# jpe17/TwoTowerMLRetrieval

Hardware: AMD Instinct MI355X
Metric: queries/sec top-k over 10M x 256-d docs (higher is better)
Workload: dtype f32 results (bit-identical to the fp32 FMA chain); f16-MFMA screen + fp32 rescoring; 1 GPU; exact cosine top-10 of B=1024 queries over 10000000 x 256 fp32 unit-norm passages resident in HBM (BASELINE configs[3]; configs[1] batch), row-sharded over 1 GPU(s), screened path (f16-MFMA filter + exact fp32 rescoring, bit-identical to the fp32 kernel); n_docs=10000000, dim=256, batch=1024, k=10, parallelism=rowshard1

## Files before the change

twotowermlretrieval_amd/csrc/screen.hip:

```cpp
#include "score_topk.h"
#include "keep_word.h"
#include <cmath>

#include <hip/hip_fp16.h>
#include <limits.h>
#include <math.h>

namespace {

typedef _Float16 h8 __attribute__((ext_vector_type(8)));
typedef _Float16 h4 __attribute__((ext_vector_type(4)));
typedef unsigned u32x4 __attribute__((ext_vector_type(4)));
typedef __attribute__((address_space(3))) void lds_void;
typedef const __attribute__((address_space(1))) void gbl_void;

#ifndef TT_SCREEN_STAGGER
#define TT_SCREEN_STAGGER 1
#endif
constexpr int SW = 8;
constexpr int STILE_BYTES = 32 * 512;
constexpr int SRING = 8;
constexpr int STPB = 2;
constexpr int SCAP = 128;
constexpr int SURV_MAX = 1024;
constexpr int POOL_MAX = 8192;
constexpr int FIN_MAX_CHUNKS = 2048;

struct SCand {
    float v;
    int x;
};

__device__ __forceinline__ float screen_eps(float qnorm, float dmax)
{
    return 1.10e-3f * qnorm * dmax + 1e-6f * (qnorm + dmax);
}

template <int NCH>
__device__ __forceinline__ void bf16_to_f16_lds(char *base, int lane)
{
    uint4 v[NCH];
#pragma unroll
    for (int i = 0; i < NCH; ++i)
        v[i] = *(const uint4 *)(base + (i * 64 + lane) * 16);
#pragma unroll
    for (int i = 0; i < NCH; ++i) {
        unsigned w[4] = {v[i].x, v[i].y, v[i].z, v[i].w};
#pragma unroll
        for (int e = 0; e < 4; ++e) {
            const _Float16 lo = (_Float16)__uint_as_float(w[e] << 16);
            const _Float16 hi = (_Float16)__uint_as_float(w[e] & 0xffff0000u);
            w[e] = (unsigned)__builtin_bit_cast(unsigned short, lo) | ((unsigned)__builtin_bit_cast(unsigned short, hi) << 16);
        }
        *(uint4 *)(base + (i * 64 + lane) * 16) = uint4{w[0], w[1], w[2], w[3]};
    }
}

__device__ __forceinline__ SCand scand_load_l2(const SCand *p)
{
    unsigned long long u = __hip_atomic_load((const unsigned long long *)p, __ATOMIC_RELAXED, __HIP_MEMORY_SCOPE_AGENT);
    SCand c;
    c.v = __uint_as_float((unsigned)u);
    c.x = (int)(u >> 32);
    return c;
}

struct ScreenParams {
    const float *Q;
    const _Float16 *D16;
    int B, N, k;
    int n_chunks, tiles_per_chunk, n_tiles;
    int static_tiles, tail_g, tail_blocks;
    int *tail_ctr;
    float dmax;
    SCand *cand;
    int *pcnt;
    int *flag;
    float *max_val;
    const float *thr0;
    int thr0_stride;
    const h8 *qimg;
    const float *qnorm;
    const float *dbg_thr;
    const unsigned *keep;
};

__device__ __forceinline__ void scand_store_async(const SCand *base, unsigned byte_off, float v, int x)
{
    const unsigned long long bits = ((unsigned long long)(unsigned)x << 32) | (unsigned long long)__float_as_uint(v);
    asm volatile("global_store_dwordx2 %0, %1, %2\n\ts_nop 1" ::"v"(byte_off), "v"(bits), "s"(base) : "memory");
}

__device__ __forceinline__ void f32_store_async(float *dst, float v)
{
    asm volatile("global_store_dword %0, %1, off\n\ts_nop 0" ::"v"(dst), "v"(v) : "memory");
}

constexpr int SQUART = SCAP / 4;
constexpr int SQ_TRIGGER = SQUART - 10;
constexpr int SQ_KEEP_MAX = 4 * SQ_TRIGGER - 4;

__device__ __forceinline__ void screen_compact(SCand *base, const int (&n)[4], int k, float slack, int lane, int &n_new,
                                               float &thr_new, bool &have, bool &overflow)
{
    float v[2];
    int x[2], rank[2];
    bool live[2];
#pragma unroll
    for (int i = 0; i < 2; ++i) {
        v[i] = -INFINITY;
        x[i] = INT_MAX;
        rank[i] = 0;
        live[i] = (lane & 31) < ((lane >> 5) ? n[2 * i + 1] : n[2 * i]);
        if (live[i]) {
            const SCand c = scand_load_l2(base + 64 * i + lane);
            v[i] = c.v;
            x[i] = c.x;
        }
    }
#pragma unroll
    for (int i2 = 0; i2 < 2; ++i2) {
#pragma unroll
        for (int sub = 0; sub < 2; ++sub) {
            const int lim = n[2 * i2 + sub];
            for (int l2 = 0; l2 < lim; ++l2) {
                const float sv = __builtin_bit_cast(float, __builtin_amdgcn_readlane(__builtin_bit_cast(int, v[i2]), 32 * sub + l2));
                const int sx = __builtin_amdgcn_readlane(x[i2], 32 * sub + l2);
#pragma unroll
                for (int i = 0; i < 2; ++i)
                    rank[i] += (sv > v[i] || (sv == v[i] && sx < x[i])) ? 1 : 0;
            }
        }
    }
    const int total = n[0] + n[1] + n[2] + n[3];
    have = total >= k;
    overflow = false;
    n_new = total;
    thr_new = -INFINITY;
    if (have) {
        float kth = -INFINITY;
#pragma unroll
        for (int i = 0; i < 2; ++i) {
            const unsigned long long bk = __ballot(live[i] && rank[i] == k - 1);
            if (bk)
                kth = __builtin_bit_cast(float, __builtin_amdgcn_readlane(__builtin_bit_cast(int, v[i]), __ffsll((long long)bk) - 1));
        }
        thr_new = kth - slack;
        n_new = 0;
#pragma unroll
        for (int i = 0; i < 2; ++i)
            n_new += __popcll(__ballot(live[i] && v[i] >= thr_new));
        if (n_new > SQ_KEEP_MAX) {
            overflow = true;
            n_new = k;
        }
    }
#pragma unroll
    for (int i = 0; i < 2; ++i)
        if (live[i] && rank[i] < n_new) {
            SCand c;
            c.v = v[i];
            c.x = x[i];
            base[SQUART * (rank[i] & 3) + (rank[i] >> 2)] = c;
        }
}

__global__ __launch_bounds__(128) void q_image_kernel(const float *__restrict__ Q, int B, h8 *__restrict__ img,
                                                      float *__restrict__ qnorm, int *__restrict__ flag, int n_flags,
                                                      int *__restrict__ tail_ctr, int n_ctr)
{
    __shared__ int any_bad[2];
    if (blockIdx.x == 0)
        for (int i = threadIdx.x; i < n_ctr; i += 128)
            tail_ctr[i] = 0;
    const int lane = threadIdx.x & 63, wv = threadIdx.x >> 6;
    const int S = blockIdx.x * 2 + wv;
    const int g = lane >> 4, n = lane & 15;
    const int qrow = 16 * S + n;
    const bool live = qrow < B;
    const float *qp = Q + (size_t)min(qrow, B - 1) * 256 + 8 * g;
    float ss = 0.0f;
    bool bad = false;
#pragma unroll
    for (int s = 0; s < 8; ++s) {
        const f32x4 a = *(const f32x4 *)(qp + 32 * s);
        const f32x4 b = *(const f32x4 *)(qp + 32 * s + 4);
        h8 hv;
#pragma unroll
        for (int e = 0; e < 4; ++e) {
            const float x0 = live ? a[e] : 0.0f, x1 = live ? b[e] : 0.0f;
            ss += x0 * x0 + x1 * x1;
            bad |= !(fabsf(x0) <= 60000.0f) || !(fabsf(x1) <= 60000.0f);
            hv[e] = (_Float16)x0;
            hv[4 + e] = (_Float16)x1;
        }
        img[((size_t)S * 8 + s) * 64 + lane] = hv;
    }
    ss += __shfl_xor(ss, 16);
    ss += __shfl_xor(ss, 32);
    if (g == 0)
        qnorm[qrow] = sqrtf(ss);
    const bool wave_bad = __ballot(bad && live) != 0ull;
    if (lane == 0)
        any_bad[wv] = wave_bad ? 1 : 0;
    __syncthreads();
    if (threadIdx.x == 0 && (int)blockIdx.x < n_flags)
        flag[blockIdx.x] = (any_bad[0] | any_bad[1]) ? 2 : 0;
}

template <bool MAXONLY, int NSET, bool BF = false, bool MASKED = false>
__global__ __launch_bounds__(SW * 64, 2) void screen_kernel(ScreenParams p)
{
    extern __shared__ __attribute__((aligned(16))) char ring[];
    constexpr int DMA_AUX = NSET < 3 ? 2 : 0;
    const int lane = threadIdx.x & 63;
    const int w = __builtin_amdgcn_readfirstlane(threadIdx.x >> 6);
    const int chunk = blockIdx.x % p.n_chunks;
    const int qgroup = blockIdx.x / p.n_chunks;
    int t0 = chunk * p.tiles_per_chunk;
    int t1 = min(t0 + p.tiles_per_chunk, p.static_tiles);
    __shared__ int next_block;
    const int k = p.k;
    const int g = lane >> 4, n = lane & 15;
    constexpr int QW = 16 * NSET, QB = SW * QW;
    const int qbase = qgroup * QB + w * QW;
    const bool wave_live = qbase < p.B;

    h8 qreg[NSET][8];
    float eps2[NSET];
    f32x4 negthr[NSET];
    int cnt[NSET];
#pragma unroll
    for (int c = 0; c < NSET; ++c)
        cnt[c] = 0;
#pragma unroll
    for (int c = 0; c < NSET; ++c) {
        const int qrow = qbase + 16 * c + n;
        const bool live = qrow < p.B;
        float qn = 0.0f;
        if (wave_live) {
            const h8 *src = p.qimg + ((size_t)(qbase / 16 + c) * 8) * 64 + lane;
#pragma unroll
            for (int s = 0; s < 8; ++s)
                qreg[c][s] = src[s * 64];
            qn = p.qnorm[qrow];
        }
        eps2[c] = 2.0f * screen_eps(qn, p.dmax);
        const float floor_thr = -(1.01f * qn * p.dmax + 1e-30f);
        const float t_init = live ? ((!MAXONLY && p.thr0) ? fmaxf(p.thr0[(size_t)qrow * p.thr0_stride + p.thr0_stride - 1] - eps2[c], floor_thr)
                                                    : floor_thr)
                            : INFINITY;
        float c_init = -t_init;
        if (MAXONLY)
            c_init = (p.dbg_thr && live) ? -p.dbg_thr[qrow] : 0.0f;
        negthr[c] = f32x4{c_init, c_init, c_init, c_init};
    }

    SCand *const cwave = p.cand + ((size_t)blockIdx.x * QB + w * QW) * SCAP;

    auto compact_where = [&](int c, unsigned qmask) {
        asm volatile("s_waitcnt vmcnt(0)" ::: "memory");
        while (qmask) {
            const int q = __ffs((int)qmask) - 1;
            qmask &= qmask - 1;
            const int nq[4] = {__builtin_amdgcn_readlane(cnt[c], q), __builtin_amdgcn_readlane(cnt[c], q + 16),
                               __builtin_amdgcn_readlane(cnt[c], q + 32), __builtin_amdgcn_readlane(cnt[c], q + 48)};
            const float slack = __builtin_bit_cast(float, __builtin_amdgcn_readlane(__builtin_bit_cast(int, eps2[c]), q));
            int n_new;
            float tn;
            bool have, ovf;
            screen_compact(cwave + (size_t)(16 * c + q) * SCAP, nq, k, slack, lane, n_new, tn, have, ovf);
            if (ovf && lane == 0)
                atomicOr(p.flag + ((qbase + 16 * c) >> 5), 1);
            if (n == q) {
                cnt[c] = (n_new - g + 3) >> 2;
                if (have)
                    negthr[c] = f32x4{-tn, -tn, -tn, -tn};
            }
        }
    };

    const char *D = (const char *)p.D16;
    const char *rowp[2];
    auto set_rows = [&](int tile) {
#pragma unroll
        for (int i = 0; i < 2; ++i) {
            const int row = 2 * (2 * w + i) + (lane >> 5);
            const int doc = min(tile * 32 + row, p.N - 1);
            const int chunk16 = (lane & 31) ^ (row & 15);
            rowp[i] = D + (size_t)doc * 512 + chunk16 * 16;
        }
    };
    auto dma_issue = [&](int tile, int stage) {
        set_rows(min(tile, t1 - 1));
        char *dst = ring + stage * STILE_BYTES + (2 * w) * 1024;
        __builtin_amdgcn_global_load_lds((gbl_void *)rowp[0], (lds_void *)dst, 16, 0, DMA_AUX);
        __builtin_amdgcn_global_load_lds((gbl_void *)rowp[1], (lds_void *)(dst + 1024), 16, 0, DMA_AUX);
    };
    auto dma_piece = [&](int i, int stage) {
        char *dst = ring + stage * STILE_BYTES + (2 * w + i) * 1024;
        __builtin_amdgcn_global_load_lds((gbl_void *)rowp[i], (lds_void *)dst, 16, 0, DMA_AUX);
    };

    for (;;) {
    if (t0 < t1) {
#pragma unroll
        for (int gi = 0; gi < SRING - STPB; ++gi)
            dma_issue(t0 + gi, gi);
        int stage = 0;
        const int rd_base = n * 512;
        f32x4 acc[2][NSET];
        const bool late = TT_SCREEN_STAGGER && w >= 4;
        bool pending = false;
        int ptile = 0;
        unsigned pkw = 0xffffffffu;
        auto epilogue = [&](int tile, unsigned kw) {
                const int tile_base = tile * 32;
            const bool partial = tile_base + 32 > p.N;
            const bool holes = MASKED && kw != 0xffffffffu;
            const unsigned kwg = MASKED ? kw >> (4 * g) : 0xffffffffu;
            auto dropped = [&](int u, int r) {
                return tile_base + 16 * u + 4 * g + r >= p.N || (MASKED && ((kwg >> (16 * u + r)) & 1u) == 0u);
            };
            if (!MAXONLY) {
                if (partial || holes) {
#pragma unroll
                    for (int u = 0; u < 2; ++u)
#pragma unroll
                        for (int r = 0; r < 4; ++r)
                            if (dropped(u, r)) {
#pragma unroll
                                for (int c = 0; c < NSET; ++c)
                                    acc[u][c][r] = -INFINITY;
                            }
                }
                int mall = INT_MIN;
#pragma unroll
                for (int u = 0; u < 2; ++u)
#pragma unroll
                    for (int c = 0; c < NSET; ++c)
#pragma unroll
                        for (int r = 0; r < 4; ++r)
                            mall = max(mall, __float_as_int(acc[u][c][r]));
                if (__ballot(mall >= 0) != 0ull) {
#pragma unroll
                    for (int c = 0; c < NSET; ++c) {
                        int mu[2];
#pragma unroll
                        for (int u = 0; u < 2; ++u)
                            mu[u] = max(max(__float_as_int(acc[u][c][0]), __float_as_int(acc[u][c][1])),
                                        max(__float_as_int(acc[u][c][2]), __float_as_int(acc[u][c][3])));
                        if (__ballot(max(mu[0], mu[1]) >= 0) == 0ull)
                            continue;
                        const unsigned mine = (unsigned)(((16 * c + n) * SCAP + SQUART * g) * sizeof(SCand));
                        const float thr_c = -negthr[c][0];
#pragma unroll
                        for (int u = 0; u < 2; ++u) {
                            if (__ballot(mu[u] >= 0) == 0ull)
                                continue;
#pragma unroll
                            for (int r = 0; r < 4; ++r) {
                                if (__float_as_int(acc[u][c][r]) >= 0) {
                                    scand_store_async(cwave, mine + (unsigned)cnt[c] * (unsigned)sizeof(SCand),
                                                      acc[u][c][r] + thr_c, tile_base + 16 * u + 4 * g + r);
                                    ++cnt[c];
                                }
                            }
                        }
                        unsigned long long full = __ballot(cnt[c] > SQ_TRIGGER);
                        full = (full | (full >> 32));
                        full = (full | (full >> 16)) & 0xffffull;
                        if (full)
                            compact_where(c, (unsigned)full);
                    }
                }
            } else {
#pragma unroll
                for (int c = 0; c < NSET; ++c) {
                    float m = -INFINITY;
                    if (!partial && !holes) {
                        int mi = INT_MIN;
#pragma unroll
                        for (int u = 0; u < 2; ++u)
#pragma unroll
                            for (int r = 0; r < 4; ++r)
                                mi = max(mi, __float_as_int(acc[u][c][r]));
                        m = __int_as_float(mi);
                    } else {
#pragma unroll
                        for (int u = 0; u < 2; ++u)
#pragma unroll
                            for (int r = 0; r < 4; ++r)
                                m = fmaxf(m, !dropped(u, r) ? acc[u][c][r] : -INFINITY);
                    }
                    m = fmaxf(m, __shfl_xor(m, 16));
                    m = fmaxf(m, __shfl_xor(m, 32));
                    const int qrow = qbase + 16 * c + n;
                    if (g == 0 && qrow < p.B)
                        f32_store_async(p.max_val + (size_t)qrow * p.n_tiles + tile, m);
                }
            }
                };
        for (int tile = t0; tile < t1; ++tile) {
            if ((tile - t0) % STPB == 0) {
                asm volatile("s_waitcnt vmcnt(%0)" ::"n"(2 * (SRING - 2 * STPB)) : "memory");
                if (BF && tile == t0) {
#pragma unroll
                    for (int i = 0; i < STPB; ++i)
                        bf16_to_f16_lds<2>(ring + ((stage + i) % SRING) * STILE_BYTES + (2 * w) * 1024, lane);
                    asm volatile("s_waitcnt lgkmcnt(0)" ::: "memory");
                }
                __builtin_amdgcn_s_barrier();
            } else if (BF && (tile - t0) % STPB == STPB - 1) {
                asm volatile("s_waitcnt vmcnt(%0)" ::"n"(2 * (SRING - 3 * STPB + 1)) : "memory");
#pragma unroll
                for (int i = 1; i <= STPB; ++i)
                    bf16_to_f16_lds<2>(ring + ((stage + i) % SRING) * STILE_BYTES + (2 * w) * 1024, lane);
                asm volatile("s_waitcnt lgkmcnt(0)" ::: "memory");
            }
            const int fill_stage = (stage + SRING - STPB) % SRING;
            set_rows(min(tile + SRING - STPB, t1 - 1));
            if (!wave_live) {
                dma_piece(0, fill_stage);
                dma_piece(1, fill_stage);
            }
            if (wave_live) {
                if (late && pending)
                    epilogue(ptile, pkw);
                const char *buf = ring + stage * STILE_BYTES + rd_base;
                h8 a0[3], a1[3];
                auto a_read = [&](int s) {
                    const int off = ((4 * s + g) ^ n) << 4;
                    a0[s % 3] = *(const h8 *)(buf + off);
                    a1[s % 3] = *(const h8 *)(buf + 16 * 512 + off);
                };
                a_read(0);
                a_read(1);
                unsigned kw = 0xffffffffu;
#pragma unroll
                for (int s = 0; s < 8; ++s) {
                    if (s + 2 < 8)
                        a_read(s + 2);
                    if (MASKED && s == 0)
                        keep_word_issue(p.keep + __builtin_amdgcn_readfirstlane(tile), kw, a0[0]);
                    if (s == 2)
                        dma_piece(0, fill_stage);
                    if (s == 6)
                        dma_piece(1, fill_stage);
                    __builtin_amdgcn_sched_barrier(0);
#pragma unroll
                    for (int c = 0; c < NSET; ++c) {
                        const f32x4 c0 = s == 0 ? negthr[c] : acc[0][c];
                        const f32x4 c1 = s == 0 ? negthr[c] : acc[1][c];
                        acc[0][c] = __builtin_amdgcn_mfma_f32_16x16x32_f16(a0[s % 3], qreg[c][s], c0, 0, 0, 0);
                        acc[1][c] = __builtin_amdgcn_mfma_f32_16x16x32_f16(a1[s % 3], qreg[c][s], c1, 0, 0, 0);
                    }
                    __builtin_amdgcn_sched_barrier(0);
                }
                if (MASKED)
                    keep_word_wait(kw, acc[1][NSET - 1]);
                if (late) {
                    pending = true;
                    ptile = tile;
                    pkw = kw;
                } else {
                    epilogue(tile, kw);
                }
            }
            stage = (stage + 1) % SRING;
        }
        if (wave_live && late && pending)
            epilogue(ptile, pkw);
    }
    if (MAXONLY || p.tail_blocks == 0)
        break;
    asm volatile("s_waitcnt vmcnt(0)" ::: "memory");
    __builtin_amdgcn_s_barrier();
    if (threadIdx.x == 0)
        next_block = atomicAdd(p.tail_ctr + qgroup, 1);
    __syncthreads();
    const int blk = next_block;
    if (blk >= p.tail_blocks)
        break;
    t0 = p.static_tiles + blk * p.tail_g;
    t1 = min(t0 + p.tail_g, p.n_tiles);
    }
    asm volatile("s_waitcnt vmcnt(0)" ::: "memory");
    __builtin_amdgcn_s_barrier();

    if (MAXONLY)
        return;
#pragma unroll
    for (int c = 0; c < NSET; ++c) {
        int tot = cnt[c] + __shfl_xor(cnt[c], 16);
        tot += __shfl_xor(tot, 32);
        const unsigned long long over = __ballot(tot > k) & 0xffffull;
        if (over)
            compact_where(c, (unsigned)over);
        int packed = cnt[c] << (8 * g);
        packed |= __shfl_xor(packed, 16);
        packed |= __shfl_xor(packed, 32);
        const int qrow = qbase + 16 * c + n;
        if (g == 0 && qrow < p.B)
            p.pcnt[(size_t)qrow * p.n_chunks + chunk] = packed;
    }
}

constexpr int TW = 4;
constexpr int TSLAB_BYTES = 32 * 128;
constexpr int TSTAGE = 4;
constexpr int TDMA = 4;
constexpr int TSTREAM_AUX = 2;

template <bool MAXONLY, int NQS = 2, bool BF = false, bool MASKED = false>
__global__ __launch_bounds__(TW * 64, 2) void screen_stream_kernel(ScreenParams p)
{
    constexpr int QPT = 16 * NQS;
    extern __shared__ __attribute__((aligned(16))) char ring_all[];
    const int lane = threadIdx.x & 63;
    const int w = __builtin_amdgcn_readfirstlane(threadIdx.x >> 6);
    char *const ring = ring_all + w * (TSTAGE * TSLAB_BYTES);
    const int task = blockIdx.x * TW + w;
    const int n_qtiles = (p.B + QPT - 1) / QPT;
    if (task >= n_qtiles * p.n_chunks)
        return;
    const int qtile = task / p.n_chunks, chunk = task % p.n_chunks;
    const int t0 = chunk * p.tiles_per_chunk;
    const int t1 = min(t0 + p.tiles_per_chunk, p.n_tiles);
    const int k = p.k;
    const int g = lane >> 4, n = lane & 15;
    const int qbase = qtile * QPT;

    h8 qreg[NQS][8];
    float eps2[NQS];
    f32x4 negthr[NQS];
    int cnt[NQS];
#pragma unroll
    for (int c = 0; c < NQS; ++c) {
        cnt[c] = 0;
        const int qrow = qbase + 16 * c + n;
        const bool live = qrow < p.B;
        const h8 *src = p.qimg + ((size_t)(qbase / 16 + c) * 8) * 64 + lane;
#pragma unroll
        for (int s = 0; s < 8; ++s)
            qreg[c][s] = src[s * 64];
        const float qn = p.qnorm[qrow];
        eps2[c] = 2.0f * screen_eps(qn, p.dmax);
        const float floor_thr = -(1.01f * qn * p.dmax + 1e-30f);
        const float t_init = live ? ((!MAXONLY && p.thr0) ? fmaxf(p.thr0[(size_t)qrow * p.thr0_stride + p.thr0_stride - 1] - eps2[c], floor_thr)
                                                    : floor_thr)
                            : INFINITY;
        float c_init = -t_init;
        if (MAXONLY)
            c_init = (p.dbg_thr && live) ? -p.dbg_thr[qrow] : 0.0f;
        negthr[c] = f32x4{c_init, c_init, c_init, c_init};
    }

    SCand *const cwave = p.cand + (size_t)task * QPT * SCAP;

    auto compact_where = [&](int c, unsigned qmask) {
        asm volatile("s_waitcnt vmcnt(0)" ::: "memory");
        while (qmask) {
            const int q = __ffs((int)qmask) - 1;
            qmask &= qmask - 1;
            const int nq[4] = {__builtin_amdgcn_readlane(cnt[c], q), __builtin_amdgcn_readlane(cnt[c], q + 16),
                               __builtin_amdgcn_readlane(cnt[c], q + 32), __builtin_amdgcn_readlane(cnt[c], q + 48)};
            const float slack = __builtin_bit_cast(float, __builtin_amdgcn_readlane(__builtin_bit_cast(int, eps2[c]), q));
            int n_new;
            float tn;
            bool have, ovf;
            screen_compact(cwave + (size_t)(16 * c + q) * SCAP, nq, k, slack, lane, n_new, tn, have, ovf);
            if (ovf && lane == 0)
                atomicOr(p.flag + ((qbase + 16 * c) >> 5), 1);
            if (n == q) {
// ... 105 lines not shown
                        const float thr_c = -negthr[c][0];
#pragma unroll
                        for (int u = 0; u < 2; ++u)
#pragma unroll
                            for (int r = 0; r < 4; ++r) {
                                if (__float_as_int(acc[u][c][r]) >= 0) {
                                    scand_store_async(cwave, mine + (unsigned)cnt[c] * (unsigned)sizeof(SCand),
                                                      acc[u][c][r] + thr_c, tile_base + 16 * u + 4 * g + r);
                                    ++cnt[c];
                                }
                            }
                        unsigned long long full = __ballot(cnt[c] > SQ_TRIGGER);
                        full = (full | (full >> 32));
                        full = (full | (full >> 16)) & 0xffffull;
                        if (full)
                            compact_where(c, (unsigned)full);
                    }
                }
            } else {
#pragma unroll
                for (int c = 0; c < NQS; ++c) {
                    float m = -INFINITY;
#pragma unroll
                    for (int u = 0; u < 2; ++u)
#pragma unroll
                        for (int r = 0; r < 4; ++r)
                            m = fmaxf(m, ((!partial && !holes) || !dropped(u, r)) ? acc[u][c][r] : -INFINITY);
                    m = fmaxf(m, __shfl_xor(m, 16));
                    m = fmaxf(m, __shfl_xor(m, 32));
                    const int qrow = qbase + 16 * c + n;
                    if (g == 0 && qrow < p.B)
                        f32_store_async(p.max_val + (size_t)qrow * p.n_tiles + tile, m);
                }
            }
        }
    }
    asm volatile("s_waitcnt vmcnt(0)" ::: "memory");
    if (MAXONLY)
        return;
#pragma unroll
    for (int c = 0; c < NQS; ++c) {
        int tot = cnt[c] + __shfl_xor(cnt[c], 16);
        tot += __shfl_xor(tot, 32);
        const unsigned long long over = __ballot(tot > k) & 0xffffull;
        if (over)
            compact_where(c, (unsigned)over);
        int packed = cnt[c] << (8 * g);
        packed |= __shfl_xor(packed, 16);
        packed |= __shfl_xor(packed, 32);
        const int qrow = qbase + 16 * c + n;
        if (g == 0 && qrow < p.B)
            p.pcnt[(size_t)qrow * p.n_chunks + chunk] = packed;
    }
}

struct FinishParams {
    const float *Q;
    const float *D32;
    const unsigned *Dbf;
    int B, N, k, n_chunks;
    float dmax;
    const SCand *cand;
    const int *pcnt;
    int *flag;
    int64_t idx_offset;
    float *out_val;
    int64_t *out_idx;
    int q_per_block;
    int *stats;
};

__device__ __forceinline__ bool before_f(float sa, int ia, float sb, int ib) { return sa > sb || (sa == sb && ia < ib); }

__device__ __forceinline__ unsigned f32_order_key(float f)
{
    const unsigned b = __float_as_uint(f);
    return (b & 0x80000000u) ? ~b : (b | 0x80000000u);
}
__device__ __forceinline__ float f32_from_order_key(unsigned k)
{
    return __uint_as_float((k & 0x80000000u) ? (k & 0x7fffffffu) : ~k);
}

__global__ __launch_bounds__(256) void screen_finish_kernel(FinishParams p)
{
    __shared__ float pool_v[POOL_MAX];
    __shared__ float qs[256];
    __shared__ float sv_v[SURV_MAX];
    __shared__ int sv_x[SURV_MAX];
    __shared__ float red_v[4];
    __shared__ int hist[256];
    extern __shared__ int fin_dyn[];
    int *const ccnt = fin_dyn;
    int *const pre = fin_dyn + p.n_chunks;
    __shared__ int sel[2];
    __shared__ int n_pool, n_surv;
    const int row = blockIdx.x, tid = threadIdx.x;
    if (tid == 0)
        n_pool = n_surv = 0;
    qs[tid] = p.Q[(size_t)row * 256 + tid];
    __syncthreads();
    float ss = qs[tid] * qs[tid];
#pragma unroll
    for (int off = 32; off >= 1; off >>= 1)
        ss += __shfl_xor(ss, off);
    if ((tid & 63) == 0)
        red_v[tid >> 6] = ss;
    __syncthreads();
    const float eps2 = 2.0f * screen_eps(sqrtf(red_v[0] + red_v[1] + red_v[2] + red_v[3]), p.dmax);
    __syncthreads();

    const int qgroup = row / p.q_per_block, qin = row % p.q_per_block;
    bool too_many = false;
    const int per = (p.n_chunks + 255) / 256;
    {
        int sum = 0;
        for (int c = tid * per; c < min(tid * per + per, p.n_chunks); ++c) {
            const int v = p.pcnt[(size_t)row * p.n_chunks + c];
            ccnt[c] = v;
            sum += (v & 0xff) + ((v >> 8) & 0xff) + ((v >> 16) & 0xff) + ((v >> 24) & 0xff);
        }
        int inc = sum;
#pragma unroll
        for (int off = 1; off < 64; off <<= 1) {
            const int v = __shfl_up(inc, off);
            if ((tid & 63) >= off)
                inc += v;
        }
        if ((tid & 63) == 63)
            hist[tid >> 6] = inc;
        __syncthreads();
        int base = 0;
        for (int wv = 0; wv < (tid >> 6); ++wv)
            base += hist[wv];
        if (tid == 255)
            n_pool = base + inc;
        __syncthreads();
        hist[tid] = base + inc - sum;
    }
    __syncthreads();
    {
        int run = hist[tid];
        for (int c = tid * per; c < min(tid * per + per, p.n_chunks); ++c) {
            pre[c] = run;
            const int v = ccnt[c];
            run += (v & 0xff) + ((v >> 8) & 0xff) + ((v >> 16) & 0xff) + ((v >> 24) & 0xff);
        }
        if (tid == 255)
            pre[p.n_chunks] = n_pool;
    }
    __syncthreads();
    const int total = n_pool;
    if (total > POOL_MAX)
        too_many = true;
    auto locate = [&](int m) -> const SCand * {
        int lo = 0, hi = p.n_chunks;
        while (hi - lo > 1) {
            const int mid = (lo + hi) >> 1;
            if (pre[mid] <= m)
                lo = mid;
            else
                hi = mid;
        }
        int o = m - pre[lo], slot = 0;
#pragma unroll
        for (int gq = 0; gq < 4; ++gq) {
            const int ng = (ccnt[lo] >> (8 * gq)) & 0xff;
            if (o >= 0 && o < ng)
                slot = SQUART * gq + o;
            o -= ng;
            if (o < 0)
// ... 150 lines not shown
                hv[e] = (_Float16)v[e];
            }
            *(h4 *)(out + row * d + x) = hv;
        }
#pragma unroll
        for (int off = 32; off >= 1; off >>= 1)
            ss += __shfl_xor(ss, off);
        nmax = fmaxf(nmax, sqrtf(ss));
    }
#pragma unroll
    for (int off = 32; off >= 1; off >>= 1)
        amax = fmaxf(amax, __shfl_xor(amax, off));
    if (lane == 0) {
        red[wave] = nmax;
        red[4 + wave] = amax;
    }
    __syncthreads();
    if (threadIdx.x == 0) {
        atomicMax(stats, __float_as_uint(fmaxf(fmaxf(red[0], red[1]), fmaxf(red[2], red[3]))));
        atomicMax(stats + 1, __float_as_uint(fmaxf(fmaxf(red[4], red[5]), fmaxf(red[6], red[7]))));
    }
}

__global__ __launch_bounds__(256) void build_from_bf16_kernel(const unsigned short *__restrict__ S, int64_t N, int d,
                                                              float *__restrict__ out32, _Float16 *__restrict__ out16,
                                                              unsigned *__restrict__ stats)
{
    __shared__ float red[8];
    const int lane = threadIdx.x & 63, wave = threadIdx.x >> 6;
    float nmax = 0.0f, amax = 0.0f;
    for (int64_t row = (int64_t)blockIdx.x * 4 + wave; row < N; row += (int64_t)gridDim.x * 4) {
        float ss = 0.0f;
        for (int x = lane * 4; x < d; x += 256) {
            const uint2 raw = *(const uint2 *)(S + row * d + x);
            f32x4 v;
            v[0] = __uint_as_float(raw.x << 16);
            v[1] = __uint_as_float(raw.x & 0xffff0000u);
            v[2] = __uint_as_float(raw.y << 16);
            v[3] = __uint_as_float(raw.y & 0xffff0000u);
            h4 hv;
#pragma unroll
            for (int e = 0; e < 4; ++e) {
                ss += v[e] * v[e];
                amax = fmaxf(amax, fabsf(v[e]));
                if (!(fabsf(v[e]) <= 3.0e38f))
                    amax = INFINITY;
                hv[e] = (_Float16)v[e];
            }
            if (out32)
                *(f32x4 *)(out32 + row * d + x) = v;
            if (out16)
                *(h4 *)(out16 + row * d + x) = hv;
        }
#pragma unroll
        for (int off = 32; off >= 1; off >>= 1)
            ss += __shfl_xor(ss, off);
        nmax = fmaxf(nmax, sqrtf(ss));
    }
#pragma unroll
    for (int off = 32; off >= 1; off >>= 1)
        amax = fmaxf(amax, __shfl_xor(amax, off));
    if (lane == 0) {
        red[wave] = nmax;
        red[4 + wave] = amax;
    }
    __syncthreads();
    if (threadIdx.x == 0 && stats) {
        atomicMax(stats, __float_as_uint(fmaxf(fmaxf(red[0], red[1]), fmaxf(red[2], red[3]))));
        atomicMax(stats + 1, __float_as_uint(fmaxf(fmaxf(red[4], red[5]), fmaxf(red[6], red[7]))));
    }
}

struct SPlan {
    bool stream;
    int nset;
    int n_qgroups;
    int q_per_block;
    int n_tiles, n_chunks, tiles_per_chunk;
    int static_tiles, tail_g, tail_blocks;
    size_t tailctr_off;
    bool sample;
    int s_tiles, s_chunks, s_tiles_per_chunk;
    int64_t s_docs;
    size_t cand_off, pcnt_off, smax_val_off, sthr_val_off, qimg_off, qnorm_off, stats_off, ws_bytes;
    int rows_pad;
};

constexpr int64_t SAMPLE_MIN_N = 65536;
constexpr int STREAM_MAX_B = 64;

int one_round(bool stream, int n_qgroups)
{
    return stream ? (tt_device_cus() * 2 * TW + n_qgroups - 1) / n_qgroups : (tt_device_cus() + n_qgroups - 1) / n_qgroups;
}

SPlan make_splan(int B, int64_t N, int k)
{
    SPlan pl;
    pl.stream = B <= STREAM_MAX_B;
    if (B <= SW * 32) {
        pl.nset = B <= SW * 16 ? 1 : 2;
    } else {
        const int groups = (B + SW * 64 - 1) / (SW * 64);
        pl.nset = (B + groups - 1) / groups <= SW * 48 ? 3 : 4;
    }
    pl.q_per_block = pl.stream ? (B <= 32 ? 32 : 64) : SW * 16 * pl.nset;
    pl.n_qgroups = (B + pl.q_per_block - 1) / pl.q_per_block;
    pl.n_tiles = (int)((N + 31) / 32);
    int max_chunks = pl.stream && N >= SAMPLE_MIN_N ? FIN_MAX_CHUNKS : POOL_MAX / (k + 16);
    if (!pl.stream)
        max_chunks = max_chunks > 255 ? 255 : max_chunks;
    const TTChunks c = tt_chunks(pl.n_tiles, one_round(pl.stream, pl.n_qgroups), max_chunks);
    pl.n_chunks = c.n_chunks;
    const TTTailSplit t = tt_tail_split(c.tiles_per_chunk, c.n_chunks, pl.n_tiles,
                                        pl.stream ? 0 : TT_AB_SWITCH(TT_SCREEN_TAIL_DIV, 8), 16, 8, 32);
    pl.tiles_per_chunk = t.own;
    pl.static_tiles = t.static_tiles;
    pl.tail_g = t.tail_g;
    pl.tail_blocks = t.tail_blocks;
    const int n_tasks = pl.n_qgroups * pl.n_chunks;
    const size_t rows = (size_t)pl.n_qgroups * pl.q_per_block;
    pl.rows_pad = (int)rows;
    pl.sample = N >= SAMPLE_MIN_N;
    int64_t s_docs = N / 64;
    const int per_k = k <= 16 ? 4096 : 2048;
    const int64_t s_min = (int64_t)k * per_k < N / 4 ? (int64_t)k * per_k : N / 4;
    s_docs = s_docs < s_min ? s_min : s_docs;
    s_docs = s_docs < 32 ? 32 : s_docs;
    pl.s_docs = (s_docs + 31) / 32 * 32;
    pl.s_tiles = (int)(pl.s_docs / 32);
    const TTChunks sc = tt_chunks(pl.s_tiles, one_round(pl.stream, pl.n_qgroups), INT_MAX);
    pl.s_tiles_per_chunk = sc.tiles_per_chunk;
    pl.s_chunks = pl.sample ? sc.n_chunks : 0;
    TTWorkspace ws;
    pl.cand_off = ws.take((size_t)n_tasks * pl.q_per_block * SCAP * sizeof(SCand));
    pl.pcnt_off = ws.take(rows * pl.n_chunks * sizeof(int));
    pl.smax_val_off = ws.take(rows * (size_t)(pl.sample ? pl.s_tiles : 1) * sizeof(float));
    pl.sthr_val_off = ws.take(rows * sizeof(float));
    pl.qimg_off = ws.take(rows * 256 * sizeof(_Float16));
    pl.qnorm_off = ws.take(rows * sizeof(float));
    pl.tailctr_off = ws.take((size_t)pl.n_qgroups * sizeof(int));
    pl.stats_off = ws.take(rows * 2 * sizeof(int));
    pl.ws_bytes = ws.off;
    return pl;
}

template <bool MAXONLY, bool BF, bool MASKED>
const void *screen_fn(bool stream, int q_per_block, int nset)
{
    if (stream)
        return q_per_block == 64 ? (const void *)screen_stream_kernel<MAXONLY, 4, BF, MASKED>
                                 : (const void *)screen_stream_kernel<MAXONLY, 2, BF, MASKED>;
    switch (nset) {
    case 4: return (const void *)screen_kernel<MAXONLY, 4, BF, MASKED>;
    case 3: return (const void *)screen_kernel<MAXONLY, 3, BF, MASKED>;
    case 2: return (const void *)screen_kernel<MAXONLY, 2, BF, MASKED>;
    default: return (const void *)screen_kernel<MAXONLY, 1, BF, MASKED>;
    }
}

template <bool MAXONLY, bool BF>
const void *screen_fn(bool stream, int q_per_block, int nset, bool masked)
{
    return masked ? screen_fn<MAXONLY, BF, true>(stream, q_per_block, nset) : screen_fn<MAXONLY, BF, false>(stream, q_per_block, nset);
}

int launch_screen(bool stream, int q_per_block, int nset, bool maxonly, ScreenParams p, int n_tasks, hipStream_t st,
                  bool bf16 = false, bool masked = false)
{
    const void *fn = maxonly ? (bf16 ? screen_fn<true, true>(stream, q_per_block, nset, masked) : screen_fn<true, false>(stream, q_per_block, nset, masked))
                             : (bf16 ? screen_fn<false, true>(stream, q_per_block, nset, masked) : screen_fn<false, false>(stream, q_per_block, nset, masked));
    const size_t lds = stream ? (size_t)TW * TSTAGE * TSLAB_BYTES : (size_t)SRING * STILE_BYTES;
    const int blocks = stream ? (n_tasks + TW - 1) / TW : n_tasks;
    TT_HIP_CHECK(hipFuncSetAttribute(fn, hipFuncAttributeMaxDynamicSharedMemorySize, (int)lds));
    void *args[] = {&p};
    TT_HIP_CHECK(hipLaunchKernel(fn, dim3(blocks), dim3((stream ? TW : SW) * 64), args, lds, st));
    return TT_OK;
}

}

TT_EXPORT int tt_index_build_f16(const float *D, int64_t N, int d, void *D16, float *stats, tt_stream_t stream)
{
    if (N < 0 || d <= 0 || (d & 3))
        return tt_fail(TT_ERR_BAD_SHAPE, "tt_index_build_f16: N=%lld d=%d", (long long)N, d);
    if (!stats || (N > 0 && (!D || !D16)))
        return tt_fail(TT_ERR_BAD_SHAPE, "tt_index_build_f16: null pointer");
    hipStream_t st = (hipStream_t)stream;
    TT_RC_CHECK(tt_zero_async(stats, 2 * sizeof(float), st));
    if (N == 0)
        return TT_OK;
    const int64_t want_blocks = (N + 3) / 4;
    hipLaunchKernelGGL(build_f16_kernel, dim3((unsigned)(want_blocks > 8192 ? 8192 : want_blocks)), dim3(256), 0, st, D,
                       N, d, (_Float16 *)D16, (unsigned *)stats);
    TT_LAUNCH_CHECK();
    return TT_OK;
}

TT_EXPORT int tt_index_build_from_bf16(const void *D_bf16, int64_t N, int d, float *D32, void *D16, float *stats,
                                       int reset_stats, tt_stream_t stream)
{
    if (N < 0 || d <= 0 || (d & 3))
        return tt_fail(TT_ERR_BAD_SHAPE, "tt_index_build_from_bf16: N=%lld d=%d", (long long)N, d);
    if (N > 0 && (!D_bf16 || !D32))
        return tt_fail(TT_ERR_BAD_SHAPE, "tt_index_build_from_bf16: null pointer");
    hipStream_t st = (hipStream_t)stream;
    if (stats && reset_stats)
        TT_RC_CHECK(tt_zero_async(stats, 2 * sizeof(float), st));
    if (N == 0)
        return TT_OK;
    const int64_t want_blocks = (N + 3) / 4;
    hipLaunchKernelGGL(build_from_bf16_kernel, dim3((unsigned)(want_blocks > 8192 ? 8192 : want_blocks)), dim3(256), 0,
                       st, (const unsigned short *)D_bf16, N, d, D32, (_Float16 *)D16, (unsigned *)stats);
    TT_LAUNCH_CHECK();
    return TT_OK;
}

TT_EXPORT size_t tt_score_topk_screened_workspace_bytes(int B, int64_t N, int d, int k)
{
    if (B <= 0 || N <= 0)
        return 0;
    return make_splan(B, N, k).ws_bytes + tt_score_topk_workspace_bytes(B, N, d, k);
}

TT_EXPORT size_t tt_score_topk_screened_stats_offset(int B, int64_t N, int d, int k)
{
    (void)d;
    if (B <= 0 || N <= 0)
        return 0;
    return make_splan(B, N, k).stats_off;
}

namespace {
__global__ void seed_fill_kernel(float *seed, int n)
{
    const int i = blockIdx.x * 256 + threadIdx.x;
    if (i < n)
        seed[i] = -3.0e38f;
}

enum class Phase {
    Whole,
    SeedThreshold,
    SeedList,
    Seeded,
};

int screened_impl(const char *who, Phase phase, const float *Q, int B, int d, const void *D32, const void *D16, int64_t N, int k,
                  int k_seed, float dmax_norm, int64_t idx_offset, float *out_val, int64_t *out_idx, int32_t *fallback_flag,
                  float *seed, void *workspace, size_t workspace_bytes, void *const *prof_events, hipStream_t st,
                  bool bf16 = false, const unsigned *keep = nullptr)
{
    if (B <= 0 || N <= 0 || k <= 0)
        return tt_fail(TT_ERR_BAD_SHAPE, "%s: B=%d N=%lld k=%d", who, B, (long long)N, k);
    if (d != 256)
        return tt_fail(TT_ERR_UNSUPPORTED, "%s: d=%d (supported: 256)", who, d);
    if (k > 64)
        return tt_fail(TT_ERR_UNSUPPORTED, "%s: k=%d > 64", who, k);
    if (N >= (int64_t)INT_MAX - 64)
        return tt_fail(TT_ERR_UNSUPPORTED, "%s: N too large; shard the corpus", who);
    if (!(dmax_norm >= 0.0f) || !(dmax_norm < 60000.0f))
        return tt_fail(TT_ERR_UNSUPPORTED, "%s: corpus norm %g outside the fp16 range", who, dmax_norm);
    const bool seed_only = phase == Phase::SeedThreshold || phase == Phase::SeedList;
    const bool caller_seed = phase == Phase::Seeded;
    if (!Q || !D16 || !fallback_flag || (!seed_only && (!D32 || !out_val || !out_idx)) || (phase != Phase::Whole && !seed))
        return tt_fail(TT_ERR_BAD_SHAPE, "%s: null pointer", who);
    if (seed_only && (k_seed < 1 || k_seed > k))
        return tt_fail(TT_ERR_BAD_SHAPE, "%s: k_seed=%d outside [1, k=%d]", who, k_seed, k);
    if ((uintptr_t)keep & 3)
        return tt_fail(TT_ERR_BAD_SHAPE, "%s: keep must be 4-byte aligned", who);
    const SPlan pl = make_splan(B, N, k);
    const size_t need = pl.ws_bytes + (bf16 ? tt_score_topk_bf16_workspace_bytes(B, N, d, k) : tt_score_topk_workspace_bytes(B, N, d, k));
    if (!workspace || workspace_bytes < need || ((uintptr_t)workspace & 255) || (bf16 && ((uintptr_t)D16 & 15)))
        return tt_fail(TT_ERR_WORKSPACE, "%s: workspace %zu < %zu bytes", who, workspace_bytes, need);
    char *ws = (char *)workspace;
    const int k_thr = phase == Phase::SeedThreshold ? k_seed : k;
    float *thr_out = phase == Phase::SeedThreshold ? seed : (float *)(ws + pl.sthr_val_off);

    ScreenParams sp;
    sp.Q = Q;
    sp.D16 = (const _Float16 *)D16;
    sp.B = B;
    sp.N = (int)N;
    sp.k = k;
    sp.n_chunks = pl.n_chunks;
    sp.tiles_per_chunk = pl.tiles_per_chunk;
    sp.n_tiles = pl.n_tiles;
    sp.static_tiles = pl.static_tiles;
    sp.tail_g = pl.tail_g;
    sp.tail_blocks = pl.tail_blocks;
    sp.tail_ctr = (int *)(ws + pl.tailctr_off);
    sp.dmax = dmax_norm;
    sp.cand = (SCand *)(ws + pl.cand_off);
    sp.pcnt = (int *)(ws + pl.pcnt_off);
    sp.flag = fallback_flag;
    sp.max_val = nullptr;
    sp.thr0 = nullptr;
    sp.thr0_stride = k;
    sp.qimg = (const h8 *)(ws + pl.qimg_off);
    sp.qnorm = (const float *)(ws + pl.qnorm_off);
    sp.dbg_thr = nullptr;
    sp.keep = keep;
    const bool masked = keep != nullptr;
    if (caller_seed) {
        sp.thr0 = seed;
        sp.thr0_stride = 1;
    } else {
        hipLaunchKernelGGL(q_image_kernel, dim3(pl.rows_pad / 32), dim3(128), 0, st, Q, B, (h8 *)(ws + pl.qimg_off),
                           (float *)(ws + pl.qnorm_off), fallback_flag, (B + 31) / 32, (int *)(ws + pl.tailctr_off),
                           pl.n_qgroups);
        TT_LAUNCH_CHECK();
        if (pl.sample) {
            ScreenParams ss = sp;
            ss.N = (int)pl.s_docs;
            ss.n_tiles = pl.s_tiles;
            ss.n_chunks = pl.s_chunks;
            ss.tiles_per_chunk = pl.s_tiles_per_chunk;
            ss.static_tiles = pl.s_tiles;
            ss.tail_blocks = 0;
            ss.max_val = (float *)(ws + pl.smax_val_off);
            TT_RC_CHECK(launch_screen(pl.stream, pl.q_per_block, pl.nset, true, ss, pl.n_qgroups * pl.s_chunks, st, bf16, masked));
            if (phase == Phase::SeedList)
                TT_RC_CHECK(tt_k_largest_list(ss.max_val, B, pl.s_tiles, k_seed, seed, st));
            else
                TT_RC_CHECK(tt_kth_largest(ss.max_val, B, pl.s_tiles, k_thr, thr_out, st));
            sp.thr0 = (const float *)(ws + pl.sthr_val_off);
            sp.thr0_stride = 1;
        } else if (seed_only) {
            const int n = phase == Phase::SeedList ? B * k_seed : B;
            hipLaunchKernelGGL(seed_fill_kernel, dim3((n + 255) / 256), dim3(256), 0, st, seed, n);
            TT_LAUNCH_CHECK();
        }
    }
    if (seed_only)
        return TT_OK;
    if (prof_events)
        TT_HIP_CHECK(hipEventRecord((hipEvent_t)prof_events[0], st));
    TT_RC_CHECK(launch_screen(pl.stream, pl.q_per_block, pl.nset, false, sp, pl.n_qgroups * pl.n_chunks, st, bf16, masked));
    if (prof_events)
        TT_HIP_CHECK(hipEventRecord((hipEvent_t)prof_events[1], st));

    FinishParams fp;
    fp.Q = Q;
    fp.D32 = bf16 ? nullptr : (const float *)D32;
    fp.Dbf = bf16 ? (const unsigned *)D32 : nullptr;
    fp.B = B;
    fp.N = (int)N;
    fp.k = k;
    fp.n_chunks = pl.n_chunks;
    fp.q_per_block = pl.q_per_block;
    fp.dmax = dmax_norm;
    fp.cand = sp.cand;
    fp.pcnt = sp.pcnt;
    fp.flag = fallback_flag;
    fp.idx_offset = idx_offset;
    fp.out_val = out_val;
    fp.out_idx = out_idx;
    fp.stats = (int *)(ws + pl.stats_off);
    hipLaunchKernelGGL(screen_finish_kernel, dim3(B), dim3(256), (size_t)(2 * pl.n_chunks + 1) * sizeof(int), st, fp);
    TT_LAUNCH_CHECK();
    if (masked)
        return tt_score_topk_masked_pred(Q, B, d, D32, bf16, N, keep, k, idx_offset, out_val, out_idx, ws + pl.ws_bytes,
                                         workspace_bytes - pl.ws_bytes, fallback_flag, st);
    if (bf16)
        return tt_score_topk_bf16_pred(Q, B, d, D32, N, k, idx_offset, out_val, out_idx, ws + pl.ws_bytes,
                                       workspace_bytes - pl.ws_bytes, fallback_flag, st);
    return tt_score_topk_f32_pred(Q, B, d, (const float *)D32, N, k, idx_offset, out_val, out_idx, ws + pl.ws_bytes,
                                  workspace_bytes - pl.ws_bytes, fallback_flag, st);
}
}

TT_EXPORT size_t tt_score_topk_screened_bf16_workspace_bytes(int B, int64_t N, int d, int k)
{
    if (B <= 0 || N <= 0)
        return 0;
    return make_splan(B, N, k).ws_bytes + tt_score_topk_bf16_workspace_bytes(B, N, d, k);
}

TT_EXPORT int tt_index_stats_bf16(const void *D_bf16, int64_t N, int d, float *stats, int reset_stats, tt_stream_t stream)
{
    hipStream_t st = (hipStream_t)stream;
    if (N < 0 || d <= 0 || d % 4 != 0 || d > 4096)
        return tt_fail(TT_ERR_BAD_SHAPE, "tt_index_stats_bf16: N=%lld d=%d", (long long)N, d);
    if (!stats || (N > 0 && !D_bf16))
        return tt_fail(TT_ERR_BAD_SHAPE, "tt_index_stats_bf16: null pointer");
    if (reset_stats)
        TT_RC_CHECK(tt_zero_async(stats, 2 * sizeof(float), st));
    if (N == 0)
        return TT_OK;
    const int64_t want_blocks = (N + 3) / 4;
    hipLaunchKernelGGL(build_from_bf16_kernel, dim3((unsigned)(want_blocks > 8192 ? 8192 : want_blocks)), dim3(256), 0,
                       st, (const unsigned short *)D_bf16, N, d, (float *)nullptr, (_Float16 *)nullptr, (unsigned *)stats);
    TT_LAUNCH_CHECK();
    return TT_OK;
}

TT_EXPORT int tt_score_topk_screened_bf16(const float *Q, int B, int d, const void *D_bf16, int64_t N, int k, float dmax_norm,
                                          int64_t idx_offset, float *out_val, int64_t *out_idx, int32_t *fallback_flag,
                                          void *workspace, size_t workspace_bytes, void *const *prof_events, tt_stream_t stream)
{
    return screened_impl("tt_score_topk_screened_bf16", Phase::Whole, Q, B, d, D_bf16, D_bf16, N, k, k, dmax_norm, idx_offset,
                         out_val, out_idx, fallback_flag, nullptr, workspace, workspace_bytes, prof_events, (hipStream_t)stream,
                         true);
}

TT_EXPORT int tt_score_topk_screened_seed_list_bf16(const float *Q, int B, int d, const void *D_bf16, int64_t N, int k,
                                                    int k_seed, float dmax_norm, int32_t *fallback_flag, float *seed_list,
                                                    void *workspace, size_t workspace_bytes, tt_stream_t stream)
// ... 98 lines not shown
                                                       void *workspace, size_t workspace_bytes, void *const *prof_events,
                                                       tt_stream_t stream)
{
    return screened_impl("tt_score_topk_screened_seeded_masked_f32", Phase::Seeded, Q, B, d, D32, D16, N, k, k, dmax_norm,
                         idx_offset, out_val, out_idx, fallback_flag, (float *)seed, workspace, workspace_bytes, prof_events,
                         (hipStream_t)stream, false, keep);
}

TT_EXPORT int tt_score_topk_screened_seeded_masked_bf16(const float *Q, int B, int d, const void *D_bf16, int64_t N,
                                                        const uint32_t *keep, int k, float dmax_norm, int64_t idx_offset,
                                                        float *out_val, int64_t *out_idx, int32_t *fallback_flag,
                                                        const float *seed, void *workspace, size_t workspace_bytes,
                                                        void *const *prof_events, tt_stream_t stream)
{
    return screened_impl("tt_score_topk_screened_seeded_masked_bf16", Phase::Seeded, Q, B, d, D_bf16, D_bf16, N, k, k, dmax_norm,
                         idx_offset, out_val, out_idx, fallback_flag, (float *)seed, workspace, workspace_bytes, prof_events,
                         (hipStream_t)stream, true, keep);
}

namespace {
struct DbgPlan {
    int q_per_block, n_qgroups, rows_pad, n_tiles, n_chunks, tiles_per_chunk;
    size_t qimg_off, qnorm_off, flag_off, total;
};
bool make_dbg_plan(int B, int64_t N, int form, DbgPlan &pl)
{
    if (form != 0 && form != 1 && form != 2 && form != 4)
        return false;
    pl.q_per_block = form == 0 ? 32 : SW * 16 * form;
    pl.n_qgroups = (B + pl.q_per_block - 1) / pl.q_per_block;
    pl.rows_pad = pl.n_qgroups * pl.q_per_block;
    pl.n_tiles = (int)((N + 31) / 32);
    const TTChunks c = tt_chunks(pl.n_tiles, one_round(form == 0, pl.n_qgroups), INT_MAX);
    pl.tiles_per_chunk = c.tiles_per_chunk;
    pl.n_chunks = c.n_chunks;
    TTWorkspace ws;
    pl.qimg_off = ws.take((size_t)pl.rows_pad * 256 * sizeof(_Float16));
    pl.qnorm_off = ws.take((size_t)pl.rows_pad * sizeof(float));
    pl.flag_off = ws.take((size_t)(pl.rows_pad / 32 + 1) * sizeof(int));
    pl.total = ws.off;
    return true;
}
}

TT_EXPORT size_t tt_debug_screen_s16_workspace_bytes(int B, int64_t N, int form)
{
    DbgPlan pl;
    if (B <= 0 || N <= 0 || !make_dbg_plan(B, N, form, pl))
        return 0;
    return pl.total;
}

namespace {
int debug_screen(const float *Q, int B, const void *D16, int64_t N, float dmax_norm, const float *thr, int form, float *out_t,
                 void *workspace, size_t workspace_bytes, tt_stream_t stream, bool bf16)
{
    hipStream_t st = (hipStream_t)stream;
    DbgPlan pl;
    if (B <= 0 || N <= 0 || N >= (int64_t)INT_MAX - 64 || !make_dbg_plan(B, N, form, pl))
        return tt_fail(TT_ERR_BAD_SHAPE, "tt_debug_screen_s16: B=%d N=%lld form=%d", B, (long long)N, form);
    if (!Q || !D16 || !out_t)
        return tt_fail(TT_ERR_BAD_SHAPE, "tt_debug_screen_s16: null pointer");
    if (!workspace || workspace_bytes < pl.total || ((uintptr_t)workspace & 255))
        return tt_fail(TT_ERR_WORKSPACE, "tt_debug_screen_s16: workspace %zu < %zu bytes", workspace_bytes, pl.total);
    char *ws = (char *)workspace;
    ScreenParams sp;
    sp.Q = Q;
    sp.D16 = (const _Float16 *)D16;
    sp.B = B;
    sp.N = (int)N;
    sp.k = 1;
    sp.n_chunks = pl.n_chunks;
    sp.tiles_per_chunk = pl.tiles_per_chunk;
    sp.n_tiles = pl.n_tiles;
    sp.static_tiles = pl.n_tiles;
    sp.tail_g = 1;
    sp.tail_blocks = 0;
    sp.tail_ctr = nullptr;
    sp.dmax = dmax_norm;
    sp.cand = nullptr;
    sp.pcnt = nullptr;
    sp.flag = (int *)(ws + pl.flag_off);
    sp.max_val = out_t;
    sp.thr0 = nullptr;
    sp.thr0_stride = 1;
    sp.qimg = (const h8 *)(ws + pl.qimg_off);
    sp.qnorm = (const float *)(ws + pl.qnorm_off);
    sp.dbg_thr = thr;
    sp.keep = nullptr;
    hipLaunchKernelGGL(q_image_kernel, dim3(pl.rows_pad / 32), dim3(128), 0, st, Q, B, (h8 *)(ws + pl.qimg_off),
                       (float *)(ws + pl.qnorm_off), sp.flag, pl.rows_pad / 32, (int *)nullptr, 0);
    TT_LAUNCH_CHECK();
    return launch_screen(form == 0, pl.q_per_block, form, true, sp, pl.n_qgroups * pl.n_chunks, st, bf16);
}
}

TT_EXPORT int tt_debug_screen_s16(const float *Q, int B, const void *D16, int64_t N, float dmax_norm, const float *thr,
                                  int form, float *out_t, void *workspace, size_t workspace_bytes, tt_stream_t stream)
{
    return debug_screen(Q, B, D16, N, dmax_norm, thr, form, out_t, workspace, workspace_bytes, stream, false);
}

TT_EXPORT int tt_debug_screen_s16_bf16(const float *Q, int B, const void *D_bf16, int64_t N, float dmax_norm, const float *thr,
                                       int form, float *out_t, void *workspace, size_t workspace_bytes, tt_stream_t stream)
{
    return debug_screen(Q, B, D_bf16, N, dmax_norm, thr, form, out_t, workspace, workspace_bytes, stream, true);
}
```

Measured before the change: 263,600 queries/s.

## Keep per-chunk top-2 sample maxima in registers instead of per-tile HBM writes

In the sampling pass, each lane now holds a running top-2 of per-tile maxima in registers across its chunk, with no cross-lane shuffle or global store per tile. It writes only 4*STOP values per query per chunk at the end, and the kth-largest/seed selection then reads this smaller array, which is aliased onto the candidate buffer. The aim is to cut global write traffic and selection work in the threshold-seeding step. The finish kernel also reuses pool_v for survivor values and gains an occupancy hint to cut LDS use. The risk is a looser threshold estimate: keeping only the top 2 per lane-group per chunk could drop tiles that would otherwise have counted toward the kth-largest.

```diff
diff --git a/twotowermlretrieval_amd/csrc/screen.hip b/twotowermlretrieval_amd/csrc/screen.hip
--- a/twotowermlretrieval_amd/csrc/screen.hip
+++ b/twotowermlretrieval_amd/csrc/screen.hip
@@ -25,6 +25,8 @@
 constexpr int SURV_MAX = 1024;
 constexpr int POOL_MAX = 8192;
 constexpr int FIN_MAX_CHUNKS = 2048;
+constexpr int STOP = 2;
+constexpr int STOP_MIN_CHUNKS = 64;
 
 struct SCand {
     float v;
@@ -77,6 +79,7 @@
     int *pcnt;
     int *flag;
     float *max_val;
+    float *top_val;
     const float *thr0;
     int thr0_stride;
     const h8 *qimg;
@@ -208,7 +211,7 @@
         flag[blockIdx.x] = (any_bad[0] | any_bad[1]) ? 2 : 0;
 }
 
-template <bool MAXONLY, int NSET, bool BF = false, bool MASKED = false>
+template <bool MAXONLY, int NSET, bool BF = false, bool MASKED = false, bool ONCHIP = false>
 __global__ __launch_bounds__(SW * 64, 2) void screen_kernel(ScreenParams p)
 {
     extern __shared__ __attribute__((aligned(16))) char ring[];
@@ -302,6 +305,13 @@
         __builtin_amdgcn_global_load_lds((gbl_void *)rowp[i], (lds_void *)dst, 16, 0, DMA_AUX);
     };
 
+    float top[ONCHIP ? NSET : 1][STOP];
+#pragma unroll
+    for (int c = 0; c < (ONCHIP ? NSET : 1); ++c)
+#pragma unroll
+        for (int j = 0; j < STOP; ++j)
+            top[c][j] = -INFINITY;
+
     for (;;) {
     if (t0 < t1) {
 #pragma unroll
@@ -392,6 +402,16 @@
 #pragma unroll
                             for (int r = 0; r < 4; ++r)
                                 m = fmaxf(m, !dropped(u, r) ? acc[u][c][r] : -INFINITY);
+                    }
+                    if (ONCHIP) {
+#pragma unroll
+                        for (int j = 0; j < STOP; ++j) {
+                            float &t = top[ONCHIP ? c : 0][j];
+                            const float hi = fmaxf(t, m);
+                            m = fminf(t, m);
+                            t = hi;
+                        }
+                        continue;
                     }
                     m = fmaxf(m, __shfl_xor(m, 16));
                     m = fmaxf(m, __shfl_xor(m, 32));
@@ -488,8 +508,21 @@
     asm volatile("s_waitcnt vmcnt(0)" ::: "memory");
     __builtin_amdgcn_s_barrier();
 
-    if (MAXONLY)
+    if (MAXONLY) {
+        if (ONCHIP) {
+#pragma unroll
+            for (int c = 0; c < NSET; ++c) {
+                const int qrow = qbase + 16 * c + n;
+                if (qrow < p.B) {
+                    float *dst = p.top_val + ((size_t)qrow * p.n_chunks + chunk) * (4 * STOP) + g * STOP;
+#pragma unroll
+                    for (int j = 0; j < STOP; ++j)
+                        dst[j] = top[ONCHIP ? c : 0][j];
+                }
+            }
+        }
         return;
+    }
 #pragma unroll
     for (int c = 0; c < NSET; ++c) {
         int tot = cnt[c] + __shfl_xor(cnt[c], 16);
@@ -761,11 +794,11 @@
     return __uint_as_float((k & 0x80000000u) ? (k & 0x7fffffffu) : ~k);
 }
 
-__global__ __launch_bounds__(256) void screen_finish_kernel(FinishParams p)
+__global__ __launch_bounds__(256, 4) void screen_finish_kernel(FinishParams p)
 {
     __shared__ float pool_v[POOL_MAX];
     __shared__ float qs[256];
-    __shared__ float sv_v[SURV_MAX];
+    float *const sv_v = pool_v;
     __shared__ int sv_x[SURV_MAX];
     __shared__ float red_v[4];
     __shared__ int hist[256];
@@ -1082,6 +1115,8 @@
     bool sample;
     int s_tiles, s_chunks, s_tiles_per_chunk;
     int64_t s_docs;
+    bool s_onchip;
+    int s_vals;
     size_t cand_off, pcnt_off, smax_val_off, sthr_val_off, qimg_off, qnorm_off, stats_off, ws_bytes;
     int rows_pad;
 };
@@ -1132,30 +1167,34 @@
     const TTChunks sc = tt_chunks(pl.s_tiles, one_round(pl.stream, pl.n_qgroups), INT_MAX);
     pl.s_tiles_per_chunk = sc.tiles_per_chunk;
     pl.s_chunks = pl.sample ? sc.n_chunks : 0;
+    const size_t cand_bytes = (size_t)n_tasks * pl.q_per_block * SCAP * sizeof(SCand);
+    pl.s_onchip = pl.sample && !pl.stream && pl.s_chunks >= STOP_MIN_CHUNKS && TT_AB_SWITCH(TT_SCREEN_SAMPLE_ONCHIP, 1) != 0 &&
+                  rows * (size_t)pl.s_chunks * 4 * STOP * sizeof(float) <= cand_bytes;
+    pl.s_vals = pl.s_onchip ? pl.s_chunks * 4 * STOP : pl.s_tiles;
     TTWorkspace ws;
-    pl.cand_off = ws.take((size_t)n_tasks * pl.q_per_block * SCAP * sizeof(SCand));
+    pl.cand_off = ws.take(cand_bytes);
     pl.pcnt_off = ws.take(rows * pl.n_chunks * sizeof(int));
-    pl.smax_val_off = ws.take(rows * (size_t)(pl.sample ? pl.s_tiles : 1) * sizeof(float));
     pl.sthr_val_off = ws.take(rows * sizeof(float));
     pl.qimg_off = ws.take(rows * 256 * sizeof(_Float16));
     pl.qnorm_off = ws.take(rows * sizeof(float));
     pl.tailctr_off = ws.take((size_t)pl.n_qgroups * sizeof(int));
     pl.stats_off = ws.take(rows * 2 * sizeof(int));
+    pl.smax_val_off = pl.s_onchip ? pl.cand_off : ws.take(rows * (size_t)(pl.sample ? pl.s_tiles : 1) * sizeof(float));
     pl.ws_bytes = ws.off;
     return pl;
 }
 
-template <bool MAXONLY, bool BF, bool MASKED>
+template <bool MAXONLY, bool BF, bool MASKED, bool ONCHIP = false>
 const void *screen_fn(bool stream, int q_per_block, int nset)
 {
     if (stream)
         return q_per_block == 64 ? (const void *)screen_stream_kernel<MAXONLY, 4, BF, MASKED>
                                  : (const void *)screen_stream_kernel<MAXONLY, 2, BF, MASKED>;
     switch (nset) {
-    case 4: return (const void *)screen_kernel<MAXONLY, 4, BF, MASKED>;
-    case 3: return (const void *)screen_kernel<MAXONLY, 3, BF, MASKED>;
-    case 2: return (const void *)screen_kernel<MAXONLY, 2, BF, MASKED>;
-    default: return (const void *)screen_kernel<MAXONLY, 1, BF, MASKED>;
+    case 4: return (const void *)screen_kernel<MAXONLY, 4, BF, MASKED, ONCHIP>;
+    case 3: return (const void *)screen_kernel<MAXONLY, 3, BF, MASKED, ONCHIP>;
+    case 2: return (const void *)screen_kernel<MAXONLY, 2, BF, MASKED, ONCHIP>;
+    default: return (const void *)screen_kernel<MAXONLY, 1, BF, MASKED, ONCHIP>;
     }
 }
 
@@ -1165,10 +1204,19 @@
     return masked ? screen_fn<MAXONLY, BF, true>(stream, q_per_block, nset) : screen_fn<MAXONLY, BF, false>(stream, q_per_block, nset);
 }
 
+template <bool BF>
+const void *screen_onchip_fn(int nset, bool masked)
+{
+    return masked ? screen_fn<true, BF, true, true>(false, 0, nset) : screen_fn<true, BF, false, true>(false, 0, nset);
+}
+
 int launch_screen(bool stream, int q_per_block, int nset, bool maxonly, ScreenParams p, int n_tasks, hipStream_t st,
                   bool bf16 = false, bool masked = false)
 {
-    const void *fn = maxonly ? (bf16 ? screen_fn<true, true>(stream, q_per_block, nset, masked) : screen_fn<true, false>(stream, q_per_block, nset, masked))
+    if (p.top_val && (!maxonly || stream))
+        return tt_fail(TT_ERR_UNSUPPORTED, "launch_screen: top_val outside the shared-tile sample pass");
+    const void *fn = p.top_val ? (bf16 ? screen_onchip_fn<true>(nset, masked) : screen_onchip_fn<false>(nset, masked))
+                     : maxonly ? (bf16 ? screen_fn<true, true>(stream, q_per_block, nset, masked) : screen_fn<true, false>(stream, q_per_block, nset, masked))
                              : (bf16 ? screen_fn<false, true>(stream, q_per_block, nset, masked) : screen_fn<false, false>(stream, q_per_block, nset, masked));
     const size_t lds = stream ? (size_t)TW * TSTAGE * TSLAB_BYTES : (size_t)SRING * STILE_BYTES;
     const int blocks = stream ? (n_tasks + TW - 1) / TW : n_tasks;
@@ -1295,6 +1343,7 @@
     sp.pcnt = (int *)(ws + pl.pcnt_off);
     sp.flag = fallback_flag;
     sp.max_val = nullptr;
+    sp.top_val = nullptr;
     sp.thr0 = nullptr;
     sp.thr0_stride = k;
     sp.qimg = (const h8 *)(ws + pl.qimg_off);
@@ -1318,12 +1367,13 @@
             ss.tiles_per_chunk = pl.s_tiles_per_chunk;
             ss.static_tiles = pl.s_tiles;
             ss.tail_blocks = 0;
-            ss.max_val = (float *)(ws + pl.smax_val_off);
+            float *const s_val = (float *)(ws + pl.smax_val_off);
+            (pl.s_onchip ? ss.top_val : ss.max_val) = s_val;
             TT_RC_CHECK(launch_screen(pl.stream, pl.q_per_block, pl.nset, true, ss, pl.n_qgroups * pl.s_chunks, st, bf16, masked));
             if (phase == Phase::SeedList)
-                TT_RC_CHECK(tt_k_largest_list(ss.max_val, B, pl.s_tiles, k_seed, seed, st));
+                TT_RC_CHECK(tt_k_largest_list(s_val, B, pl.s_vals, k_seed, seed, st));
             else
-                TT_RC_CHECK(tt_kth_largest(ss.max_val, B, pl.s_tiles, k_thr, thr_out, st));
+                TT_RC_CHECK(tt_kth_largest(s_val, B, pl.s_vals, k_thr, thr_out, st));
             sp.thr0 = (const float *)(ws + pl.sthr_val_off);
             sp.thr0_stride = 1;
         } else if (seed_only) {
@@ -1588,6 +1638,7 @@
     sp.pcnt = nullptr;
     sp.flag = (int *)(ws + pl.flag_off);
     sp.max_val = out_t;
+    sp.top_val = nullptr;
     sp.thr0 = nullptr;
     sp.thr0_stride = 1;
     sp.qimg = (const h8 *)(ws + pl.qimg_off);
```

Result: faster. 268,700 queries/s (median of 6 runs) (+1.9%).
